# noisystreet/aither

Measured on AMD Instinct MI355X. Metric: Mcell-updates/sec per iteration (residual+LU-SGS), 256^3 block; % HBM roofline, higher is better.
Workload: dtype f64

## Files before the change

aither_amd/csrc/agx_api.hip:

```cpp
#include "agx_kernels.hpp"
#include <rccl/rccl.h>
#include <cstdarg>
#include <cstdio>
#include <cstring>
#include <cstdlib>
#include <cmath>
#include <vector>
#include <string>
#include <algorithm>

using namespace agx;

static char g_err[512] = "";
static int fail(const char* fmt, ...) {
  va_list ap;
  va_start(ap, fmt);
  vsnprintf(g_err, sizeof g_err, fmt, ap);
  va_end(ap);
  return 1;
}
#define HIPCHK(call)                                                       \
  do {                                                                     \
    hipError_t e_ = (call);                                                \
    if (e_ != hipSuccess)                                                  \
      return fail("%s failed: %s (%s:%d)", #call, hipGetErrorString(e_),   \
                  __FILE__, __LINE__);                                     \
  } while (0)
#define AGX_BY_MODE(sp, kernel, grid, block, stream, ...)                                  \
  do {                                                                                     \
    switch (agx::solver_mode_of(sp)) {                                                     \
      case 0: hipLaunchKernelGGL(kernel<0>, grid, block, 0, stream, __VA_ARGS__); break;   \
      case 1: hipLaunchKernelGGL(kernel<1>, grid, block, 0, stream, __VA_ARGS__); break;   \
      default: hipLaunchKernelGGL(kernel<2>, grid, block, 0, stream, __VA_ARGS__); break;  \
    }                                                                                      \
  } while (0)

namespace {

struct Block {
  BlockDev d;
  int global_pos = 0;
  double* slab = nullptr;
  double* d2 = nullptr;
  double* blockmat = nullptr;
  double* sweep_rec = nullptr;
  bool sweep_geo_built = false;
  bool x_planes_current = false;
  double *mg_forcing = nullptr, *mg_mres = nullptr, *mg_xsave = nullptr, *mg_nodes = nullptr;
  int* mg_tc = nullptr;
  int* mg_start = nullptr;
  double *mg_vf = nullptr, *mg_cf = nullptr;
  const void *mg_tc_key = nullptr, *mg_vf_key = nullptr, *mg_cf_key = nullptr;
  int* d2_tab = nullptr;
  std::vector<int> dstart;
  hipGraphExec_t sweep_graph[2][2][2] = {};
  int* kp_mem = nullptr;
  unsigned kp_epoch = 0;
  long d2idx(int i, int j, int k) const {
    const int ie = i + d.ng, je = j + d.ng, de = ie + je;
    return (long)(k + d.ng) * d.d2.ps + dstart[de] + je - std::max(0, de - (d.d2.Pi - 1));
  }
  bool state_is_a = true;
  agx_bc_surface* surf_dev = nullptr;
  std::vector<agx_bc_surface> surf_host;
  int* nr_off_dev = nullptr;
  double* nr_mem = nullptr;
  long nr_max = 0;
  int* wall_off_dev = nullptr;
  double* wall_mem = nullptr;
};

struct ConnSide {
  std::vector<long> h_dst, h_src;
  long n = 0;
  long* dst = nullptr;
  long* src = nullptr;
  long* dst2 = nullptr;
  long* src2 = nullptr;
};
struct Conn {
  agx_connection c;
  ConnSide side[2];
  long n_send = 0;
  long* send_src = nullptr;
  long* send_src2 = nullptr;
};

enum { G_RESID = 0, G_UPDATE = 1, G_BC = 2, G_SWEEP = 3, G_VISC = 4, G_PREPARE = 5,
       G_MRESID = 6, G_NGROUP = 7 };

// ... 26 lines not shown
  int* err_dev = nullptr;
  int* err_host = nullptr;
  double* halo_buf = nullptr;
  long halo_cap = 0;
  double* stage_buf = nullptr;
  size_t stage_cap = 0;
  double* rans_rec = nullptr;
  size_t rans_rec_cap = 0;
  bool use_gather = false;
  bool use_tile = true;
  int num_cu = 256;
  bool eager_ghosts = true;
  bool overlap = true;
  hipStream_t ov_stream = nullptr;
  hipEvent_t ov_ready = nullptr, ov_done = nullptr;
  bool visc_gather = false;
  bool visc_march = false;
  int lusgs_mode = 1;
  int spin_limit = 4000000;
  bool allow_fuse = true;
  bool fused_pending = false;
  bool use_graphs = true;
  bool sweep_records = true;
  bool sweep_three = true;
  hipStream_t cap_stream = nullptr;
  std::vector<hipStream_t> branch_streams;
  std::vector<hipEvent_t> branch_events;
  bool sweep_all_launch = true;
  BlockDev* blocks_tab = nullptr;
  BlockDev* blocks_tab_host = nullptr;
  size_t blocks_tab_n = 0;
  hipGraphExec_t sweep_graph_all[2][2][2] = {};
  bool mg_coarse = false;
  bool mres_plane_form = false;
  bool sweep_pipe = true;
  PipeJob* pipe_jobs[2] = {nullptr, nullptr};
  int* pipe_slot0 = nullptr;
  long long* pipe_progress = nullptr;
  unsigned long long* pipe_ticket = nullptr;
  size_t pipe_nblocks = 0;
  int pipe_njobs = 0, pipe_maxsteps = 0, pipe_waves = 4;
  long long pipe_launches = 0;
  bool halo_batch = true;
  bool halo_batch_required = false;
  int halo_batch_sides = 0;
  long halo_batch_nmax = 0;
  std::vector<int> halo_conn_order;
  struct HaloLevel { int first, sides; long nmax; };
  std::vector<HaloLevel> halo_levels;
  HaloSide* halo_tab_dev[5][2][2] = {};
  bool halo_tab_valid[5][2] = {};
  int halo_set[5] = {};
  HaloSide* halo_tab_host = nullptr;
  int mresid_split = 1;
  bool mresid_march = true;
  bool have_time_n = false;
  bool in_iterate = false, ghosts_prefilled = false;
  bool mres_deferred = false;
  hipEvent_t norm_event = nullptr;
  bool consn_pending = false;
  bool state_is_time_n = false;
  long fused_parts = 0;
  bool timing = false;
  std::vector<std::pair<hipEvent_t, hipEvent_t>> ev_pool;
  std::vector<std::pair<int, int>> ev_used;
  double t_ms[G_NGROUP] = {};
// ... 751 lines not shown
      }
      if (nmax > 0)
        hipLaunchKernelGGL(k_bc_faces, dim3((nmax + 255) / 256, b.nsurf), dim3(256), 0,
                           c->stream, b, c->gas, viscous, c->err_dev);
    } else {
      const long n = 4L * (b.ni + b.nj + b.nk);
      hipLaunchKernelGGL(k_bc_edges, dim3((n + 127) / 128), dim3(128), 0,
                         c->stream, b, c->gas, viscous, c->err_dev);
    }
  }
  HIPCHK(hipGetLastError());
  return 0;
}

int reduce_norms(agx_ctx* c, size_t blk_index, long nparts, NormPartial* out = nullptr) {
  if (!out) out = c->norm_out + blk_index;
  if (nparts > 4096) {
    NormPartial* tmp = c->norm_out + c->blocks.size();
    hipLaunchKernelGGL(k_norm_final, dim3(64), dim3(256), 0, c->stream, c->partials, nparts, tmp);
    hipLaunchKernelGGL(k_norm_final, dim3(1), dim3(256), 0, c->stream, tmp, 64L, out);
  } else {
    hipLaunchKernelGGL(k_norm_final, dim3(1), dim3(256), 0, c->stream,
                       c->partials, nparts, out);
  }
  HIPCHK(hipGetLastError());
  return 0;
}

int fill_ghosts(agx_ctx* c) {
  if (agx_phase_bc_faces(c)) return 1;
  if (agx_halo_exchange(c, AGX_HALO_STATE)) return 1;
  return agx_phase_bc_edges(c);
}
int update_pass(agx_ctx* c, int mode, int mm, double* l2, agx_linf* linf) {
  c->state_is_time_n = false;
  const double alpha[4] = {0.25, 1.0 / 3.0, 0.5, 1.0};
  if (mode != 2 && c->fused_pending) {
    Timer t(c, G_UPDATE);
    long off = 0;
    for (size_t n = 0; n < c->blocks.size(); ++n) {
      BlockDev& b = c->blocks[n].d;
      const MarchPlan mp = march_plan(c, b);
      hipLaunchKernelGGL(k_norm_final, dim3(1), dim3(256), 0, c->stream,
                         c->partials + off, mp.nparts, c->norm_out + n);
      off += mp.nparts;
      for (int e = 0; e < AGX_NEQ; ++e) std::swap(b.state[e], b.state2[e]);
    }
    c->halo_set[AGX_HALO_STATE] ^= 1;
    c->fused_pending = false;
    HIPCHK(hipGetLastError());
  } else {
    Timer t(c, G_UPDATE);
    for (size_t n = 0; n < c->blocks.size(); ++n) {
      const BlockDev& b = c->blocks[n].d;
      const int last = mm == c->cfg.nonlinear_iterations - 1;
#if AGX_FAST
      if (mode == 2 && b.d2.base) {
        const dim3 tg((b.ni + TT - 1) / TT, (b.nj + TT - 1) / TT, b.nk);
        hipLaunchKernelGGL(k_update_d2, tg, dim3(256), 0, c->stream, b, c->gas, c->sp, last,
                           c->partials);
        if (reduce_norms(c, n, (long)tg.x * tg.y * tg.z)) return 1;
        continue;
      }
#endif
      const dim3 grid = cell_grid(b, CELL_BLOCK);
      hipLaunchKernelGGL(k_update, grid, CELL_BLOCK, 0, c->stream, b, c->gas,
                         c->sp, mode, mode == 1 ? alpha[mm & 3] : 1.0, last,
                         c->partials);
      if (reduce_norms(c, n, (long)grid.x * grid.y * grid.z)) return 1;
    }
  }
  HIPCHK(hipMemcpyAsync(c->norm_host, c->norm_out,
                        sizeof(NormPartial) * c->blocks.size(),
                        hipMemcpyDeviceToHost, c->stream));
  if (c->mres_deferred)
    HIPCHK(hipMemcpyAsync(c->norm_host + c->blocks.size(), c->norm_out + c->blocks.size() + 64,
                          sizeof(NormPartial) * c->blocks.size(), hipMemcpyDeviceToHost,
                          c->stream));
  HIPCHK(hipMemcpyAsync(c->err_host, c->err_dev, sizeof(int),
                        hipMemcpyDeviceToHost, c->stream));
  if (c->in_iterate && c->eager_ghosts) {
    if (!c->norm_event) HIPCHK(hipEventCreateWithFlags(&c->norm_event, hipEventDisableTiming));
    HIPCHK(hipEventRecord(c->norm_event, c->stream));
    if (fill_ghosts(c)) return 1;
    c->ghosts_prefilled = true;
    HIPCHK(hipEventSynchronize(c->norm_event));
  } else {
    HIPCHK(hipStreamSynchronize(c->stream));
  }
  if (check_device_error(c)) return 1;
  for (size_t n = 0; n < c->blocks.size(); ++n) {
    const NormPartial& p = c->norm_host[n];
    const BlockDev& b = c->blocks[n].d;
// ... 24 lines not shown
  if (e != hipSuccess || ndev <= 0)
    return fail("no HIP device available (%s): the gfx950 library has no CPU "
                "path", hipGetErrorString(e));
  if (device < 0 || device >= ndev) return fail("device %d out of range", device);
  HIPCHK(hipSetDevice(device));
  agx_ctx* c = new agx_ctx();
  c->device = device;
  c->rank = rank;
  if (const char* kn = getenv("AGX_KERNEL")) {
    c->use_gather = !strcmp(kn, "gather");
    c->use_tile = !strcmp(kn, "tile");
  }
  c->allow_fuse = !(getenv("AGX_NO_FUSE") && atoi(getenv("AGX_NO_FUSE")) != 0);
  {
    int ncu = 0;
    HIPCHK(hipDeviceGetAttribute(&ncu, hipDeviceAttributeMultiprocessorCount, device));
    if (ncu > 0) c->num_cu = ncu;
    if (const char* w = getenv("AGX_WORKGROUPS")) c->num_cu = std::max(1, atoi(w));
    if (const char* w = getenv("AGX_VISC")) {
      c->visc_gather = !strcmp(w, "gather");
      c->visc_march = !strcmp(w, "march");
    }
    if (const char* w = getenv("AGX_EAGER_GHOSTS")) c->eager_ghosts = atoi(w) != 0;
    if (const char* w = getenv("AGX_OVERLAP")) c->overlap = atoi(w) != 0;
    if (const char* w = getenv("AGX_LUSGS")) c->lusgs_mode = !strcmp(w, "plane") ? 0 : 1;
    if (const char* w = getenv("AGX_SPIN_LIMIT")) c->spin_limit = std::max(1, atoi(w));
    if (const char* w = getenv("AGX_GRAPHS")) c->use_graphs = atoi(w) != 0;
    if (const char* w = getenv("AGX_SWEEP_ALL")) c->sweep_all_launch = atoi(w) != 0;
    if (const char* w = getenv("AGX_SWEEP_PIPE")) c->sweep_pipe = atoi(w) != 0;
    if (const char* w = getenv("AGX_SWEEP_THREE")) c->sweep_three = atoi(w) != 0;
    if (const char* w = getenv("AGX_SWEEP_RECORDS")) c->sweep_records = atoi(w) != 0;
    if (const char* w = getenv("AGX_MRESID_SPLIT")) c->mresid_split = std::min(64, std::max(1, atoi(w)));
    if (const char* w = getenv("AGX_MRESID")) c->mresid_march = strcmp(w, "plane") != 0;
    if (const char* w = getenv("AGX_HALO_BATCH")) {
      c->halo_batch = strcmp(w, "0") != 0;
      c->halo_batch_required = !strcmp(w, "require");
    }
  }
  HIPCHK(hipMalloc((void**)&c->err_dev, sizeof(int)));
  HIPCHK(hipMemset(c->err_dev, 0, sizeof(int)));
  HIPCHK(hipHostMalloc((void**)&c->err_host, sizeof(int)));
  *c->err_host = 0;
  *out = c;
  return 0;
}

void agx_ctx_destroy(agx_ctx* c) {
  if (!c) return;
  hipSetDevice(c->device);
  hipStreamSynchronize(c->stream);
  for (auto& b : c->blocks) {
    if (b.slab) hipFree(b.slab);
    if (b.d2) hipFree(b.d2);
    if (b.blockmat) hipFree(b.blockmat);
    if (b.sweep_rec) hipFree(b.sweep_rec);
    for (void* p : {(void*)b.mg_forcing, (void*)b.mg_mres, (void*)b.mg_xsave, (void*)b.mg_nodes,
                    (void*)b.mg_tc, (void*)b.mg_start, (void*)b.mg_vf, (void*)b.mg_cf})
      if (p) hipFree(p);
    if (b.d2_tab) hipFree(b.d2_tab);
    if (b.kp_mem) hipFree(b.kp_mem);
    for (auto& g1 : b.sweep_graph) for (auto& g2 : g1) for (auto& g3 : g2)
      if (g3) hipGraphExecDestroy(g3);
    if (b.surf_dev) hipFree(b.surf_dev);
    if (b.nr_off_dev) hipFree(b.nr_off_dev);
    if (b.nr_mem) hipFree(b.nr_mem);
    if (b.wall_off_dev) hipFree(b.wall_off_dev);
// ... 215 lines not shown
    HIPCHK(hipMemsetAsync(b.d2, 0, sizeof(double) * z.nd2 * D2_DOUBLES, c->stream));
    z.base = b.d2;
  }
  const int ci = d.ni + 2 * d.ng, cj = d.nj + 2 * d.ng, ck = d.nk + 2 * d.ng;
  if (upload_aos(c, b, g->farea_i, d.fa[0], 4, ci + 1, cj, ck, d.ng)) return 1;
  if (upload_aos(c, b, g->farea_j, d.fa[1], 4, ci, cj + 1, ck, d.ng)) return 1;
  if (upload_aos(c, b, g->farea_k, d.fa[2], 4, ci, cj, ck + 1, d.ng)) return 1;
  double* volp[1] = {d.vol};
  if (upload_aos(c, b, g->vol, volp, 1, ci, cj, ck, d.ng)) return 1;
  if (upload_aos(c, b, g->center, d.cen, 3, ci, cj, ck, d.ng)) return 1;
  const double* wsrc[3] = {g->width_i, g->width_j, g->width_k};
  for (int q = 0; q < 3; ++q) {
    double* wp[1] = {d.wid[q]};
    if (upload_aos(c, b, wsrc[q], wp, 1, ci, cj, ck, d.ng)) return 1;
  }
#if AGX_FAST
  if (d.d2.base) {
    const long n = (long)d.d2.Pi * d.d2.Pj * (d.nk + 2 * d.ng);
    hipLaunchKernelGGL(k_d2_geo, dim3((n + 255) / 256), dim3(256), 0, c->stream, d);
  }
#endif
  HIPCHK(hipGetLastError());
  if (g->wall_dist) {
    double* wp[1] = {d.wdist};
    if (upload_aos(c, b, g->wall_dist, wp, 1, ci, cj, ck, d.ng)) return 1;
  }
  *block_id = (int)c->blocks.size() - 1;
  return 0;
}

int agx_block_set_bcs(agx_ctx* c, int id, int n, const agx_bc_surface* s) {
  if (id < 0 || id >= (int)c->blocks.size()) return fail("bad block id %d", id);
  Block& b = c->blocks[id];
  for (auto& g1 : b.sweep_graph) for (auto& g2 : g1) for (auto& g3 : g2)
    if (g3) { hipGraphExecDestroy(g3); g3 = nullptr; }
  b.surf_host.assign(s, s + n);
  if (b.surf_dev) HIPCHK(hipFree(b.surf_dev));
  HIPCHK(hipMalloc((void**)&b.surf_dev, sizeof(agx_bc_surface) * (n > 0 ? n : 1)));
  HIPCHK(hipMemcpy(b.surf_dev, s, sizeof(agx_bc_surface) * n, hipMemcpyHostToDevice));
  b.d.surf = b.surf_dev;
  b.d.nsurf = n;
  b.d.nsurf_i = b.d.nsurf_j = b.d.nsurf_k = 0;
  int n_conn[6] = {0, 0, 0, 0, 0, 0}, n_other[6] = {0, 0, 0, 0, 0, 0};
  for (int q = 0; q < n; ++q) {
    const int st = surface_type(s[q]);
    if (st <= 2) b.d.nsurf_i++; else if (st <= 4) b.d.nsurf_j++; else b.d.nsurf_k++;
    const int t = s[q].bc_type;
    if (t < AGX_BC_SLIPWALL || t > AGX_BC_PERIODIC) return fail("unknown bc type %d", t);
    if (t == AGX_BC_INTERBLOCK || t == AGX_BC_PERIODIC) n_conn[st - 1]++; else n_other[st - 1]++;
    if (t == AGX_BC_VISCOUSWALL && s[q].state.is_wall_law) {
      if (AGX_NEQ == 5) return fail("wallTreatment=wallLaw needs the rans library");
    }
  }
  for (int q = 0; q < 6; ++q)
    b.d.side_conn[q] = n_conn[q] == 0 ? 0 : (n_other[q] == 0 ? 1 : 2);
  if (b.nr_off_dev) HIPCHK(hipFree(b.nr_off_dev));
  if (b.nr_mem) HIPCHK(hipFree(b.nr_mem));
  b.nr_off_dev = nullptr; b.nr_mem = nullptr; b.nr_max = 0;
  b.d.nr_off = nullptr; b.d.nr_grad = nullptr; b.d.nr_mach = nullptr;
  std::vector<int> off(n > 0 ? n : 1, -1);
  long total = 0;
  for (int q = 0; q < n; ++q) {
    const int t = s[q].bc_type;
    if (!s[q].state.is_nonreflecting || (t != AGX_BC_INLET && t != AGX_BC_PRESSURE_OUTLET)) continue;
    const int st = surface_type(s[q]);
    const int d3 = (st - 1) / 2, d1 = (d3 + 1) % 3, d2 = (d3 + 2) % 3;
// ... 131 lines not shown
      HIPCHK(hipMalloc((void**)&c->halo_tab_dev[what][set][q], sizeof(HaloSide) * sides));
  HIPCHK(hipStreamSynchronize(c->stream));
  HaloSide* g = c->halo_tab_host;
  HaloSide* p = c->halo_tab_host + sides;
  long off = 0;
  int n = 0;
  for (int cid : c->halo_conn_order) {
    auto& k = c->conns[cid];
    const agx_connection& cc = k.c;
    Block& b0 = c->blocks[cc.local_block[0]];
    Block& b1 = c->blocks[cc.local_block[1]];
    const bool z2 = halo_in_d2(b0, what);
    const long n0 = k.side[0].n, n1 = k.side[1].n;
    double* buf0 = c->halo_buf + off;
    double* buf1 = buf0 + n0 * AGX_NEQ;
    off += (n0 + n1) * AGX_NEQ;
    g[n] = HaloSide{halo_planes(b1, what), z2 ? k.side[0].src2 : k.side[0].src, n0, buf0};
    g[n + 1] = HaloSide{halo_planes(b0, what), z2 ? k.side[1].src2 : k.side[1].src, n1, buf1};
    p[n] = HaloSide{halo_planes(b0, what), z2 ? k.side[0].dst2 : k.side[0].dst, n0, buf0};
    p[n + 1] = HaloSide{halo_planes(b1, what), z2 ? k.side[1].dst2 : k.side[1].dst, n1, buf1};
    n += 2;
  }
  HIPCHK(hipMemcpyAsync(c->halo_tab_dev[what][set][0], g, sizeof(HaloSide) * sides,
                        hipMemcpyHostToDevice, c->stream));
  HIPCHK(hipMemcpyAsync(c->halo_tab_dev[what][set][1], p, sizeof(HaloSide) * sides,
                        hipMemcpyHostToDevice, c->stream));
  c->halo_tab_valid[what][set] = true;
  return 0;
}
}

int agx_setup_finalize(agx_ctx* c) {
  HIPCHK(hipSetDevice(c->device));
  const int ng = c->cfg.n_ghost;
  long max_parts = 1, max_halo = 1;
  long march_parts = 0;
  for (auto& blk : c->blocks) {
    const dim3 g = cell_grid(blk.d, CELL_BLOCK);
    max_parts = std::max(max_parts, (long)g.x * g.y * g.z);
    march_parts += march_plan(c, blk.d).nparts;
    if (blk.d.d2.base)
      max_parts = std::max(max_parts, mresid_wgs(c, blk.d));
  }
  max_parts = std::max(max_parts, march_parts);
  for (auto& k : c->conns) {
    const agx_connection& cc = k.c;
    const bool l0 = cc.rank[0] == c->rank, l1 = cc.rank[1] == c->rank;
    if (!l0 && !l1) continue;
    for (int s = 0; s < 2; ++s) {
      const bool mine = s == 0 ? l0 : l1, partner_mine = s == 0 ? l1 : l0;
      if (!mine) continue;
      const int lb = cc.local_block[s];
      if (lb < 0 || lb >= (int)c->blocks.size()) return fail("connection refers to unknown block");
      const BlockDev& br = c->blocks[lb].d;
      auto idxR = [&](int i, int j, int kk) { return br.idx(i, j, kk); };
      MapOut m;
      if (partner_mine) {
        const BlockDev& bs = c->blocks[cc.local_block[1 - s]].d;
        auto idxS = [&](int i, int j, int kk) { return bs.idx(i, j, kk); };
        build_side_map(cc, s, ng, idxR, idxS, m);
      } else {
        auto idxS = [&](int, int, int) { return 0L; };
        build_side_map(cc, s, ng, idxR, idxS, m);
        MapOut ms;
        auto idxRp = [&](int, int, int) { return 0L; };
        build_side_map(cc, 1 - s, ng, idxRp, idxR, ms);
// ... 41 lines not shown
      HIPCHK(hipHostMalloc((void**)&r.hsend, sizeof(double) * std::max<long>(r.count, 1)));
      HIPCHK(hipHostMalloc((void**)&r.hrecv, sizeof(double) * std::max<long>(r.count, 1)));
    }
    c->remote.push_back(r);
    const int s = my_side(c, c->conns[n]);
    agx_slab sl;
    sl.peer = c->conns[n].c.rank[1 - s];
    sl.tag = 0;
    bool seen = false;
    for (auto& pp : per_peer)
      if (pp.first == sl.peer) { sl.tag = pp.second++; seen = true; }
    if (!seen) per_peer.emplace_back(sl.peer, 1);
    sl.count = r.count;
    const bool hb = c->have_ex && c->ex.host_buffers;
    sl.send = hb ? r.hsend : r.send;
    sl.recv = hb ? r.hrecv : r.recv;
    c->slabs.push_back(sl);
  }
  if (c->have_ex) {
    const size_t nrec = 1 + (size_t)c->ex.nranks;
    HIPCHK(hipMalloc((void**)&c->rec_dev, sizeof(agx_ctx::NormRecord) * nrec));
    HIPCHK(hipHostMalloc((void**)&c->rec_host, sizeof(agx_ctx::NormRecord) * nrec));
  }
  c->n_partials = max_parts;
  HIPCHK(hipMalloc((void**)&c->partials, sizeof(NormPartial) * max_parts));
  const size_t nb = std::max<size_t>(c->blocks.size(), 1);
  HIPCHK(hipMalloc((void**)&c->norm_out, sizeof(NormPartial) * (2 * nb + 64)));
  HIPCHK(hipHostMalloc((void**)&c->norm_host, sizeof(NormPartial) * 2 * nb));
  c->finalized = true;
  return 0;
}

int agx_state_upload(agx_ctx* c, int id, const double* state) {
  c->ghosts_prefilled = false;
  c->state_is_time_n = false;
  if (flush_consn(c)) return 1;
  if (id < 0 || id >= (int)c->blocks.size()) return fail("bad block id %d", id);
  Block& b = c->blocks[id];
  const BlockDev& d = b.d;
  if (upload_aos(c, b, state, d.state, AGX_NEQ, d.ni + 2 * d.ng,
                 d.nj + 2 * d.ng, d.nk + 2 * d.ng, d.ng))
    return 1;
#if AGX_NEQ == 7
  hipLaunchKernelGGL(k_aux_field, dim3((d.nplane + 255) / 256), dim3(256), 0, c->stream, d,
                     c->gas, 1, d.viscp);
  HIPCHK(hipGetLastError());
#endif
  return 0;
}

static int field_info(Block& b, int field, double* const** p, int* ncomp, int* ghost) {
  BlockDev& d = b.d;
  static thread_local double* one[1];
  switch (field) {
    case AGX_FIELD_STATE: *p = d.state; *ncomp = AGX_NEQ; *ghost = 1; return 0;
    case AGX_FIELD_RESIDUAL: *p = d.resid; *ncomp = AGX_NEQ; *ghost = 0; return 0;
    case AGX_FIELD_CONS_N: *p = d.consn; *ncomp = AGX_NEQ; *ghost = 0; return 0;
    case AGX_FIELD_CONS_NM1: *p = d.consnm1; *ncomp = AGX_NEQ; *ghost = 0; return 0;
    case AGX_FIELD_UPDATE: *p = d.x; *ncomp = AGX_NEQ; *ghost = 1; return 0;
    case AGX_FIELD_DT: one[0] = d.dt; *p = one; *ncomp = 1; *ghost = 0; return 0;
    case AGX_FIELD_SPEC_RADIUS: one[0] = d.specrad; *p = one; *ncomp = 1; *ghost = 0; return 0;
    case AGX_FIELD_DIAGONAL: one[0] = d.a; *p = one; *ncomp = 1; *ghost = 0; return 0;
  }
  return 1;
}

// ... 152 lines not shown
    if (host_out[q])
      HIPCHK(hipMemcpyAsync(host_out[q], dev_out[q], sizeof(double) * count[q],
                            hipMemcpyDeviceToHost, c->stream));
  HIPCHK(hipMemcpyAsync(c->err_host, c->err_dev, sizeof(int), hipMemcpyDeviceToHost, c->stream));
  HIPCHK(hipStreamSynchronize(c->stream));
  if (*c->err_host == 4) {
    *c->err_host = 0;
    hipMemsetAsync(c->err_dev, 0, sizeof(int), c->stream);
    return fail("negative volume in PLOT3D block");
  }
  return 0;
}

int agx_nearest_wall_distance(agx_ctx* c, int64_t ncell, const double* cen, int64_t nwall,
                              const double* wall, double* dist) {
  if (ncell < 1) return 0;
  if (nwall < 1) return fail("no wall points");
  HIPCHK(hipSetDevice(c->device));
  double* buf = nullptr;
  if (stage_buffer(c, (size_t)(4 * ncell + 3 * nwall), &buf)) return 1;
  double *dc = buf, *dw = buf + 3 * ncell, *dd = dw + 3 * nwall;
  HIPCHK(hipMemcpyAsync(dc, cen, sizeof(double) * 3 * ncell, hipMemcpyHostToDevice, c->stream));
  HIPCHK(hipMemcpyAsync(dw, wall, sizeof(double) * 3 * nwall, hipMemcpyHostToDevice, c->stream));
  hipLaunchKernelGGL(k_nearest_wall, dim3((unsigned)((ncell + 255) / 256)), dim3(256), 0, c->stream,
                     (long)ncell, dc, (long)nwall, dw, dd);
  HIPCHK(hipGetLastError());
  HIPCHK(hipMemcpyAsync(dist, dd, sizeof(double) * ncell, hipMemcpyDeviceToHost, c->stream));
  HIPCHK(hipStreamSynchronize(c->stream));
  return 0;
}

int agx_field_upload(agx_ctx* c, int id, int field, const double* in) {
  x_changed(c);
  c->ghosts_prefilled = false;
  c->state_is_time_n = false;
  if (flush_consn(c)) return 1;
  if (id < 0 || id >= (int)c->blocks.size()) return fail("bad block id %d", id);
  Block& b = c->blocks[id];
  double* const* p; int nc, gh;
  if (field_info(b, field, &p, &nc, &gh)) return fail("field %d cannot be uploaded", field);
  const int g = gh ? b.d.ng : 0;
  if (upload_aos(c, b, in, p, nc, b.d.ni + 2 * g, b.d.nj + 2 * g, b.d.nk + 2 * g, g)) return 1;
  if (field == AGX_FIELD_UPDATE && b.d.d2.base) return d2_x_copy(c, b, 1);
  return 0;
}

static int implicit_begin(agx_ctx* c, int write_x);
int agx_phase_matrix_residual(agx_ctx* c, double* mr);
static int d2_x_copy(agx_ctx* c, Block& b, int to_d2);
#if AGX_FAST
static void d2_prepare(agx_ctx* c, Block& blk, int write_x, int again);
#endif
namespace {
int mg_solver_ok(agx_ctx* c) {
  if (!c->sp.implicit) return fail("multigrid: implicit time integration only");
  return 0;
}
int mg_x_to_planes(agx_ctx* c, Block& b) {
  return b.d.d2.base && !b.x_planes_current ? d2_x_copy(c, b, 0) : 0;
}
int mg_x_from_planes(agx_ctx* c, Block& b) { return b.d.d2.base ? d2_x_copy(c, b, 1) : 0; }
void mg_x_records(agx_ctx* c, Block& b) {
  if (b.d.sw_dyn)
    hipLaunchKernelGGL(k_mg_x_records, dim3((unsigned)((b.d.nplane + 255) / 256)), dim3(256), 0,
                       c->stream, b.d);
}
// ... 43 lines not shown
    b.mg_tc_key = tc;
  }
  if (vf && b.mg_vf_key != vf) {
    HIPCHK(hipStreamSynchronize(f->stream));
    if (!b.mg_vf) HIPCHK(hipMalloc((void**)&b.mg_vf, sizeof(double) * ncell));
    HIPCHK(hipMemcpy(b.mg_vf, vf, sizeof(double) * ncell, hipMemcpyHostToDevice));
    b.mg_vf_key = vf;
  }
  if (cf && b.mg_cf_key != cf) {
    HIPCHK(hipStreamSynchronize(f->stream));
    if (!b.mg_cf) HIPCHK(hipMalloc((void**)&b.mg_cf, sizeof(double) * 7 * ncell));
    HIPCHK(hipMemcpy(b.mg_cf, cf, sizeof(double) * 7 * ncell, hipMemcpyHostToDevice));
    b.mg_cf_key = cf;
  }
  if (!b.mg_tc) return fail("mg: no fine-to-coarse map for this block yet");
  m->tc = b.mg_tc;
  m->start[0] = b.mg_start;
  m->start[1] = b.mg_start + cni + 1;
  m->start[2] = m->start[1] + cnj + 1;
  m->vf = b.mg_vf;
  m->cf = b.mg_cf;
  return 0;
}
int mg_order(agx_ctx* producer, agx_ctx* consumer) {
  if (producer->stream != consumer->stream) HIPCHK(hipStreamSynchronize(producer->stream));
  return 0;
}
}

int agx_mg_restrict(agx_ctx* f, agx_ctx* cz, int blk, int what, const int32_t* tc,
                    const double* vf) {
  if (mg_check(f, cz, blk)) return 1;
  Block &bf = f->blocks[blk], &bc = cz->blocks[blk];
  if (what < AGX_MG_STATE || what > AGX_MG_FORCING) return fail("mg_restrict: bad selector %d", what);
  if (what != AGX_MG_FORCING && !vf) return fail("mg_restrict: volume weights missing");
  if (flush_consn(f) || flush_consn(cz)) return 1;
  MgMap m;
  if (mg_maps(f, bf, tc, vf, nullptr, bc.d.ni, bc.d.nj, bc.d.nk, &m)) return 1;
  if (what == AGX_MG_UPDATE && mg_x_to_planes(f, bf)) return 1;
  if (what == AGX_MG_FORCING && mg_x_to_planes(cz, bc)) return 1;
  if (mg_order(f, cz)) return 1;
  if (what == AGX_MG_STATE) {
    for (int e = 0; e < AGX_NEQ; ++e)
      HIPCHK(hipMemsetAsync(bc.d.state[e], 0, sizeof(double) * bc.d.nplane, cz->stream));
    cz->ghosts_prefilled = false;
    cz->state_is_time_n = false;
    cz->mg_coarse = true;
  } else if (what == AGX_MG_UPDATE) {
    for (int e = 0; e < AGX_NEQ; ++e)
      HIPCHK(hipMemsetAsync(bc.d.x[e], 0, sizeof(double) * bc.d.nplane, cz->stream));
  } else {
    if (!bf.d.mg_mres) return fail("mg_restrict: the fine level has no matrix residual yet");
    if (mg_planes(cz, bc, &bc.mg_forcing)) return 1;
    bc.d.mg_forcing = bc.mg_forcing;
  }
  hipLaunchKernelGGL(k_mg_restrict, cell_grid(bc.d, CELL_BLOCK), CELL_BLOCK, 0, cz->stream, bf.d,
                     bc.d, m, what);
  if (what == AGX_MG_FORCING)
    hipLaunchKernelGGL(k_mg_axmb, cell_grid(bc.d, CELL_BLOCK), CELL_BLOCK, 0, cz->stream, bc.d,
                       cz->gas, cz->sp);
  if (what == AGX_MG_UPDATE) {
    mg_x_records(cz, bc);
    if (mg_x_from_planes(cz, bc)) return 1;
  }
#if AGX_FAST
  if (what == AGX_MG_FORCING && bc.d.d2.base) d2_prepare(cz, bc, 0, 1);
#endif
  HIPCHK(hipGetLastError());
  return 0;
}

int agx_mg_matrix_residual(agx_ctx* c, double* mr) {
  if (mg_solver_ok(c)) return 1;
  for (auto& blk : c->blocks) {
    if (mg_planes(c, blk, &blk.mg_mres)) return 1;
    blk.d.mg_mres = blk.mg_mres;
    if (mg_x_to_planes(c, blk)) return 1;
  }
  c->mres_plane_form = true;
  const int rc = agx_phase_matrix_residual(c, mr);
  c->mres_plane_form = false;
  return rc;
}

int agx_mg_invert_diagonal(agx_ctx* c) { return implicit_begin(c, 0); }

int agx_mg_reset_diagonal(agx_ctx* c) {
  for (auto& blk : c->blocks) {
    HIPCHK(hipMemsetAsync(blk.d.a, 0, sizeof(double) * blk.d.nplane, c->stream));
    if (blk.d.am)
      HIPCHK(hipMemsetAsync(blk.d.am, 0, sizeof(double) * AGX_NJ * blk.d.nplane, c->stream));
    if (AGX_NEQ > 5) {
      HIPCHK(hipMemsetAsync(blk.d.a_t, 0, sizeof(double) * blk.d.nplane, c->stream));
      if (blk.d.am_t)
        HIPCHK(hipMemsetAsync(blk.d.am_t, 0, sizeof(double) * 2 * blk.d.nplane, c->stream));
    }
  }
  return 0;
}

int agx_mg_save_update(agx_ctx* c) {
  for (auto& blk : c->blocks) {
    if (mg_planes(c, blk, &blk.mg_xsave)) return 1;
    blk.d.mg_xsave = blk.mg_xsave;
    if (mg_x_to_planes(c, blk)) return 1;
    hipLaunchKernelGGL(k_mg_axpy, dim3((unsigned)((blk.d.nplane + 255) / 256)), dim3(256), 0,
                       c->stream, blk.d, 1);
  }
  HIPCHK(hipGetLastError());
  return 0;
}

int agx_mg_prolong(agx_ctx* cz, agx_ctx* f, int blk, const int32_t* tc, const double* cf) {
  if (mg_check(f, cz, blk)) return 1;
  Block &bf = f->blocks[blk], &bc = cz->blocks[blk];
  if (!bc.d.mg_xsave) return fail("mg_prolong: no saved update on the coarse level");
  if (!cf) return fail("mg_prolong: interpolation coefficients missing");
  MgMap m;
  if (mg_maps(f, bf, tc, nullptr, cf, bc.d.ni, bc.d.nj, bc.d.nk, &m)) return 1;
  const long nn = (long)(bc.d.ni + 1) * (bc.d.nj + 1) * (bc.d.nk + 1);
  if (!bc.mg_nodes) HIPCHK(hipMalloc((void**)&bc.mg_nodes, sizeof(double) * AGX_NEQ * nn));
  if (mg_x_to_planes(cz, bc) || mg_x_to_planes(f, bf)) return 1;
  hipLaunchKernelGGL(k_mg_axpy, dim3((unsigned)((bc.d.nplane + 255) / 256)), dim3(256), 0,
                     cz->stream, bc.d, 0);
  const dim3 tb = CELL_BLOCK;
  hipLaunchKernelGGL(k_mg_nodes, dim3((bc.d.ni + tb.x) / tb.x, (bc.d.nj + tb.y) / tb.y, bc.d.nk + 1),
                     tb, 0, cz->stream, bc.d, bc.mg_nodes);
  HIPCHK(hipGetLastError());
  if (mg_order(cz, f)) return 1;
  hipLaunchKernelGGL(k_mg_prolong, cell_grid(bf.d, tb), tb, 0, f->stream, bf.d, m,
                     (const double*)bc.mg_nodes, bc.d.ni, bc.d.nj, bc.d.nk);
  mg_x_records(cz, bc);
  mg_x_records(f, bf);
  if (mg_x_from_planes(cz, bc) || mg_x_from_planes(f, bf)) return 1;
  HIPCHK(hipGetLastError());
  return 0;
}

int agx_store_time_n(agx_ctx* c, int also_nm1) {
  if (flush_consn(c)) return 1;
  c->have_time_n = true;
  for (auto& blk : c->blocks)
    if (blk.nr_max > 0) c->ghosts_prefilled = false;
  static const bool lazy = !(getenv("AGX_NO_LAZY_CONSN") && atoi(getenv("AGX_NO_LAZY_CONSN")));
  c->state_is_time_n = true;
  if (lazy && !also_nm1 && !c->use_gather && all_tile_ok(c)) { c->consn_pending = true; return 0; }
  for (auto& blk : c->blocks)
    hipLaunchKernelGGL(k_store_time_n, cell_grid(blk.d, CELL_BLOCK), CELL_BLOCK,
// ... 118 lines not shown
  for (auto& blk : c->blocks)
    if (blk.nr_max > 0) {
      Timer t(c, G_BC);
      hipLaunchKernelGGL(k_nr_grads, dim3((blk.nr_max + 255) / 256, blk.d.nsurf), dim3(256), 0,
                         c->stream, blk.d, c->gas);
      HIPCHK(hipGetLastError());
    }
  return 0;
}

int agx_phase_explicit_update(agx_ctx* c, int mm, double* l2, agx_linf* linf) {
  const int mode = c->cfg.time_integration == AGX_TIME_RK4 ? 1 : 0;
  return update_pass(c, mode, mm, l2, linf);
}

static int implicit_begin(agx_ctx* c, int write_x);
#if AGX_FAST
static void d2_prepare(agx_ctx* c, Block& blk, int write_x, int again) {
  const BlockDev& b = blk.d;
  const dim3 grid((b.d2.Pi + TT - 1) / TT, (b.d2.Pj + TT - 1) / TT, b.nk + 2 * b.ng);
  hipLaunchKernelGGL(k_lusgs_prepare, grid, dim3(256), 0, c->stream, b, c->gas, c->sp,
                     write_x, write_x ? (unsigned)(++blk.kp_epoch) & 3u : 0u, again);
}
#endif
int agx_phase_implicit_begin(agx_ctx* c) { return implicit_begin(c, 1); }
static int implicit_begin(agx_ctx* c, int write_x) {
  x_changed(c);
  Timer t(c, G_PREPARE);
  c->sp.un_is_u = c->state_is_time_n ? 1 : 0;
  for (auto& blk : c->blocks) {
    const BlockDev& b = blk.d;
#if AGX_FAST
    if (b.d2.base) {
      bool conn = false;
      for (int q = 0; q < 6; ++q) conn = conn || b.side_conn[q] != 0;
      d2_prepare(c, blk, write_x && (c->sp.requires_init || conn) ? 1 : 0, 0);
      continue;
    }
#endif
    if (!c->sp.requires_init && write_x)
      hipLaunchKernelGGL(k_zero5, dim3((b.nplane + 255) / 256), dim3(256), 0,
                         c->stream, planes(b.x), b.nplane);
    hipLaunchKernelGGL(k_implicit_begin, cell_grid(b, CELL_BLOCK), CELL_BLOCK, 0,
                       c->stream, b, c->gas, c->sp, c->err_dev, write_x);
    if (b.sw_geo) {
      hipLaunchKernelGGL(k_sweep_records, dim3((unsigned)((b.nplane + 255) / 256)), dim3(256), 0,
                         c->stream, b, c->sp, blk.sweep_geo_built ? 0 : 1);
      blk.sweep_geo_built = true;
    }
  }
  HIPCHK(hipGetLastError());
  return 0;
}

int agx_phase_relax_forward(agx_ctx* c, int sweep) {
  x_changed(c);
  Timer t(c, G_SWEEP);
  const int full = sweep > 0 || c->sp.requires_init;
  bool swept = false;
  if (is_lusgs_solver(c) && pipe_sweep_applicable(c)) return lusgs_sweep_pipe(c, true, full);
  if (is_lusgs_solver(c) && plane_sweep_all_applicable(c)) return lusgs_sweep_all(c, true, full);
  for (auto& blk : c->blocks) {
    BlockDev& b = blk.d;
    if (is_lusgs_solver(c)) {
      if (lusgs_sweep(c, blk, true, full)) return 1;
      swept = true;
    } else {
      for (int e = 0; e < AGX_NEQ; ++e) std::swap(b.x[e], b.xold[e]);
      AGX_BY_MODE(c->sp, k_dplur, cell_grid(b, CELL_BLOCK), CELL_BLOCK, c->stream, b, c->gas,
// ... 437 lines not shown
```

aither_amd/csrc/agx_lusgs_kernels.hpp:

```cpp
#pragma once

namespace agx {

constexpr int TT = 32;
constexpr int TRS = TT + 2;
__device__ __forceinline__ int tile_diag_index(int li, int lj) {
  const int dd = li + lj;
  if (dd < TT) return dd * (dd + 1) / 2 + lj;
  const int r = 2 * TT - 2 - dd;
  return TT * TT - (r + 1) * (r + 2) / 2 + (lj - (dd - (TT - 1)));
}
__device__ __forceinline__ void tile_table(unsigned short* s_tab) {
  const int tid = threadIdx.x;
#pragma unroll
  for (int m = 0; m < 4; ++m) {
    const int li = tid & (TT - 1), lj = (tid >> 5) + 8 * m;
    s_tab[tile_diag_index(li, lj)] = (unsigned short)(li | (lj << 8));
  }
}

__device__ __forceinline__ double kp_tagged(double v, unsigned tag) {
  const unsigned long long u = (unsigned long long)__double_as_longlong(v);
  return __longlong_as_double((long long)((u & ~3ull) | tag));
}
// ... 16 lines not shown
#pragma unroll
  for (int d = 0; d < 3; ++d) {
    double a[4];
#pragma unroll
    for (int c = 0; c < 4; ++c) a[c] = b.fa[d][c][q];
    double ad = 0.0;
    if (e3[d] > 0) {
      const long ql = q - b.stride(d);
      const double v[3] = {b.cen[0][q] - b.cen[0][ql], b.cen[1][q] - b.cen[1][ql],
                           b.cen[2][q] - b.cen[2][ql]};
      const double dist = dot3(v, a);
      ad = dist != 0.0 ? a[3] / dist : 0.0;
    }
    z.pa(PA_F + 2 * d + 0)[p] = make_double2(a[0], a[1]);
    z.pa(PA_F + 2 * d + 1)[p] = make_double2(a[2], a[3]);
    z.ad(d)[p] = ad;
  }
}
__global__ void __launch_bounds__(256) k_d2_x_copy(BlockDev b, int to_d2, unsigned tag) {
  const D2Dev& z = b.d2;
  const long t = (long)blockIdx.x * blockDim.x + threadIdx.x;
  const long n = (long)z.Pi * z.Pj * (b.nk + 2 * b.ng);
  if (t >= n) return;
  const int ie = (int)(t % z.Pi), je = (int)((t / z.Pi) % z.Pj),
            ke = (int)(t / ((long)z.Pi * z.Pj));
  const long q = b.idx(ie - b.ng, je - b.ng, ke - b.ng);
  const long p = (long)ke * z.ps + z.pos2(ie, je);
#pragma unroll
  for (int e = 0; e < AGX_NEQ; ++e) {
    double* xp = reinterpret_cast<double*>(z.pa(PA_X + (e >> 1))) + 2 * p + (e & 1);
    if (to_d2) *xp = kp_tagged(b.x[e][q], tag);
    else b.x[e][q] = *xp;
  }
}

__global__ void __launch_bounds__(256)
k_lusgs_prepare(BlockDev b, GasDev g, SolverDev sp, int write_x, unsigned tag, int again) {
  __shared__ double sv[6][TT][TRS];
  __shared__ unsigned short s_tab[TT * TT];
  const D2Dev& z = b.d2;
  const int tid = threadIdx.x;
  tile_table(s_tab);
  const int i0 = blockIdx.x * TT, j0 = blockIdx.y * TT, ke = blockIdx.z;
  const int k = ke - b.ng;
  const int li = tid & (TT - 1);
  double bb[4][AGX_NEQ], x0[4][AGX_NEQ], ainv[4], vf[4];
#pragma unroll
  for (int m = 0; m < 4; ++m) {
    const int lj = (tid >> 5) + 8 * m;
    const int ie = i0 + li, je = j0 + lj;
    const int i = ie - b.ng, j = je - b.ng;
#pragma unroll
    for (int e = 0; e < AGX_NEQ; ++e) { bb[m][e] = 0.0; x0[m][e] = 0.0; }
    ainv[m] = 1.0;
    vf[m] = 0.0;
    double cs = 0.0;
    if (ie < z.Pi && je < z.Pj) {
      const long q = b.idx(i, j, k);
      double s[AGX_NEQ];
#pragma unroll
      for (int e = 0; e < AGX_NEQ; ++e) { s[e] = b.state[e][q]; sv[e][lj][li] = s[e]; }
      if (s[0] > 0.0) cs = sound_speed(g, s);
      if (sp.viscous) vf[m] = cell_visc_factor(g, s);
      const bool phys = i >= 0 && i < b.ni && j >= 0 && j < b.nj && k >= 0 && k < b.nk;
      if (phys) {
        double dvt = (b.vol[q] * (1.0 + sp.zeta)) / (b.dt[q] * sp.theta);
        if (sp.dual_time_cfl > 0.0) dvt += fmax(b.specrad[q], 0.0) / sp.dual_time_cfl;
        const double a = again ? b.ainv[q] : b.a[q] * sp.relax + dvt;
        b.ainv[q] = a;
        if (sp.diag_add) b.a[q] = a;
        ainv[m] = 1.0 / a;
        rhs_bf(b, g, sp, q, bb[m]);
        if (sp.requires_init) {
#pragma unroll
          for (int e = 0; e < AGX_NEQ; ++e) x0[m][e] = bb[m][e] * ainv[m];
        }
      }
    }
    sv[5][lj][li] = cs;
  }
  __syncthreads();
  long pos[4];
  int tli[4], tlj[4];
#pragma unroll
  for (int m = 0; m < 4; ++m) {
    const unsigned tl = s_tab[tid + 256 * m];
    tli[m] = tl & 0xff; tlj[m] = tl >> 8;
    const int ie = i0 + tli[m], je = j0 + tlj[m];
    pos[m] = -1;
    if (ie < z.Pi && je < z.Pj) {
      pos[m] = (long)ke * z.ps + z.pos2(ie, je);
#pragma unroll
      for (int h = 0; h < 3; ++h)
        z.pa(PA_S + h)[pos[m]] = make_double2(sv[2 * h][tlj[m]][tli[m]], sv[2 * h + 1][tlj[m]][tli[m]]);
    }
  }
  __syncthreads();
#pragma unroll
  for (int m = 0; m < 4; ++m) {
    const int lj = (tid >> 5) + 8 * m;
#pragma unroll
    for (int e = 0; e < AGX_NEQ; ++e) sv[e][lj][li] = bb[m][e];
    sv[5][lj][li] = ainv[m];
  }
  __syncthreads();
  double ai2[4];
#pragma unroll
  for (int m = 0; m < 4; ++m) {
    ai2[m] = sv[5][tlj[m]][tli[m]];
    if (pos[m] >= 0) {
#pragma unroll
      for (int h = 0; h < 3; ++h)
        z.pa(PA_B + h)[pos[m]] = make_double2(sv[2 * h][tlj[m]][tli[m]], sv[2 * h + 1][tlj[m]][tli[m]]);
    }
  }
  __syncthreads();
#pragma unroll
  for (int m = 0; m < 4; ++m) {
    const int lj = (tid >> 5) + 8 * m;
#pragma unroll
    for (int e = 0; e < AGX_NEQ; ++e) sv[e][lj][li] = x0[m][e];
    sv[5][lj][li] = vf[m];
  }
  __syncthreads();
#pragma unroll
  for (int m = 0; m < 4; ++m) {
    if (pos[m] >= 0) {
      if (write_x) {
        z.pa(PA_X + 0)[pos[m]] = make_double2(kp_tagged(sv[0][tlj[m]][tli[m]], tag),
                                              kp_tagged(sv[1][tlj[m]][tli[m]], tag));
        z.pa(PA_X + 1)[pos[m]] = make_double2(kp_tagged(sv[2][tlj[m]][tli[m]], tag),
                                              kp_tagged(sv[3][tlj[m]][tli[m]], tag));
        z.pa(PA_X + 2)[pos[m]] = make_double2(kp_tagged(sv[4][tlj[m]][tli[m]], tag), ai2[m]);
      }
      if (sp.viscous) z.vf()[pos[m]] = sv[5][tlj[m]][tli[m]];
    }
  }
}

struct KpRec {
  double dx[AGX_NEQ];
  double r1, v1[3], p1, h1;
  double r0, v0[3], p0, h0;
  double cs, vf;
};
constexpr int KP_NV = 19;
template <class G>
__device__ __forceinline__ void kp_build_rec(const G& g, const double* s, double cs,
                                             double vf, const double* dx, KpRec& r) {
  const double ke = g.hf + 0.5 * dot3(s + 1, s + 1);
  const double e0 = s[0] * ke + g.n * s[4];
  r.r0 = s[0]; r.p0 = s[4]; r.h0 = e0 + s[4]; r.cs = cs; r.vf = vf;
  const double r1 = s[0] + dx[0];
  const double ir = fast_rcp(r1);
  double v2 = 0.0;
#pragma unroll
  for (int q = 0; q < 3; ++q) {
    r.v0[q] = s[1 + q];
    r.v1[q] = fma(s[0], s[1 + q], dx[1 + q]) * ir;
    v2 = fma(r.v1[q], r.v1[q], v2);
  }
  const double e1 = e0 + dx[4];
  r.r1 = r1;
  r.p1 = (e1 - r1 * (g.hf + 0.5 * v2)) * g.inv_n;
  r.h1 = e1 + r.p1;
#pragma unroll
  for (int e = 0; e < AGX_NEQ; ++e) r.dx[e] = dx[e];
}
// ... 432 lines not shown
      KpFace ff;
      if (i > 0 || bc_is_connection(b, i, j, k, 1)) {
        kp_load_face(z, 0, own, visc, ff);
        kp_term_mem(z, g, visc, kbase + qlo, ff, true, acc);
      }
      if (j > 0 || bc_is_connection(b, i, j, k, 3)) {
        kp_load_face(z, 1, own, visc, ff);
        kp_term_mem(z, g, visc, kbase + qlo - 1, ff, true, acc);
      }
      if (k > 0 || bc_is_connection(b, i, j, k, 5)) col_term(cm, fk0, true, acc);
      if (i < b.ni - 1 || bc_is_connection(b, i + 1, j, k, 2)) {
        kp_load_face(z, 0, kbase + qup, visc, ff);
        kp_term_mem(z, g, visc, kbase + qup, ff, false, acc);
      }
      if (j < b.nj - 1 || bc_is_connection(b, i, j + 1, k, 4)) {
        kp_load_face(z, 1, kbase + qup + 1, visc, ff);
        kp_term_mem(z, g, visc, kbase + qup + 1, ff, false, acc);
      }
      if (k < b.nk - 1 || bc_is_connection(b, i, j, k + 1, 6)) col_term(cp, fk1, false, acc);
      const double a = 1.0 / b2.y;
      const double bv[AGX_NEQ] = {b0.x, b0.y, b1.x, b1.y, b2.x};
#pragma unroll
      for (int e = 0; e < AGX_NEQ; ++e) {
        const double r = -(c0.x[e] * a - acc[e] - bv[e]);
        l2[e] += r * r;
      }
      cm = c0; c0 = cp; fk0 = fk1;
    }
  }
  norm_block_fold(l2, -1.0e300, 0x7fffffffffffffffLL, partials + blockIdx.x);
}

__global__ void __launch_bounds__(256)
k_update_d2(BlockDev b, GasDev g, SolverDev sp, int last_mm, NormPartial* partials) {
  __shared__ double sv[AGX_NEQ][TT][TRS];
  __shared__ unsigned short s_tab[TT * TT];
  const D2Dev& z = b.d2;
  const int tid = threadIdx.x;
  tile_table(s_tab);
  __syncthreads();
  const int i0 = blockIdx.x * TT, j0 = blockIdx.y * TT, k = blockIdx.z;
#pragma unroll
  for (int m = 0; m < 4; ++m) {
    const unsigned tl = s_tab[tid + 256 * m];
    const int tli = tl & 0xff, tlj = tl >> 8;
    const int i = i0 + tli, j = j0 + tlj;
    if (i < b.ni && j < b.nj) {
      const long p = (long)(k + b.ng) * z.ps + z.pos2(i + b.ng, j + b.ng);
      const double2 x0 = z.pa(PA_X)[p], x1 = z.pa(PA_X + 1)[p], x2 = z.pa(PA_X + 2)[p];
      sv[0][tlj][tli] = x0.x; sv[1][tlj][tli] = x0.y; sv[2][tlj][tli] = x1.x;
      sv[3][tlj][tli] = x1.y; sv[4][tlj][tli] = x2.x;
    }
  }
  __syncthreads();
  const int li = tid & (TT - 1);
  double l2[AGX_NEQ] = {0, 0, 0, 0, 0};
  double vmax = -1.0e300;
  long long vlin = 0x7fffffffffffffffLL;
#pragma unroll
  for (int m = 0; m < 4; ++m) {
    const int lj = (tid >> 5) + 8 * m;
    const int i = i0 + li, j = j0 + lj;
    if (i < b.ni && j < b.nj) {
      const long q = b.idx(i, j, k);
      double r[AGX_NEQ], s[AGX_NEQ], du[AGX_NEQ], ns[AGX_NEQ];
      load5(b.resid, q, r);
      load5(b.state, q, s);
#pragma unroll
      for (int e = 0; e < AGX_NEQ; ++e) du[e] = sv[e][lj][li];
      update_prim_with_cons(g, s, du, ns);
      store5(b.state, q, ns);
      if (sp.bdf2 && last_mm) {
        double u[AGX_NEQ];
        load5(b.consn, q, u);
        store5(b.consnm1, q, u);
      }
      const long lin0 = (((long)k * b.nj + j) * b.ni + i) * AGX_NEQ;
#pragma unroll
      for (int e = 0; e < AGX_NEQ; ++e) {
        l2[e] += r[e] * r[e];
        if (r[e] > vmax || (r[e] == vmax && lin0 + e < vlin)) { vmax = r[e]; vlin = lin0 + e; }
      }
    }
  }
  const long bid = ((long)blockIdx.z * gridDim.y + blockIdx.y) * gridDim.x + blockIdx.x;
  norm_block_fold(l2, vmax, vlin, partials + bid);
}

}
```

Measured before the change: 1458.

## Fuse diagonal-plane state write into update and add lean LU-SGS prepare

The update kernel now also writes the new primitive state, sound speed and viscous factor into the diagonal-plane (d2) layout when the block qualifies. This lets the following LU-SGS prepare step run a lean kernel that only computes the RHS and inverse diagonal instead of re-gathering the state. The aim is to avoid a separate full prepare pass that rereads state from memory. Validity flags track when the d2 state is fresh, and the inverse diagonal is recomputed lazily on multigrid paths. The cost is more bookkeeping and a risk of using stale d2 data if a flag is not reset on some path that changes the state.

```diff
diff --git a/aither_amd/csrc/agx_api.hip b/aither_amd/csrc/agx_api.hip
--- a/aither_amd/csrc/agx_api.hip
+++ b/aither_amd/csrc/agx_api.hip
@@ -56,6 +56,8 @@
   hipGraphExec_t sweep_graph[2][2][2] = {};
   int* kp_mem = nullptr;
   unsigned kp_epoch = 0;
+  bool d2_state_ok = false;
+  bool ainv_stale = false;
   long d2idx(int i, int j, int k) const {
     const int ie = i + d.ng, je = j + d.ng, de = ie + je;
     return (long)(k + d.ng) * d.d2.ps + dstart[de] + je - std::max(0, de - (d.d2.Pi - 1));
@@ -148,6 +150,8 @@
   size_t blocks_tab_n = 0;
   hipGraphExec_t sweep_graph_all[2][2][2] = {};
   bool mg_coarse = false;
+  bool prepare_full = false;
+  bool mg_level = false;
   bool mres_plane_form = false;
   bool sweep_pipe = true;
   PipeJob* pipe_jobs[2] = {nullptr, nullptr};
@@ -965,8 +969,20 @@
   if (agx_halo_exchange(c, AGX_HALO_STATE)) return 1;
   return agx_phase_bc_edges(c);
 }
+void d2_state_stale(agx_ctx* c) {
+  for (auto& blk : c->blocks) blk.d2_state_ok = false;
+}
+bool lean_prepare_ok(const agx_ctx* c, const Block& blk) {
+  const BlockDev& b = blk.d;
+  if (!b.d2.base || c->prepare_full || c->mg_coarse || c->mg_level || c->sp.requires_init)
+    return false;
+  for (int q = 0; q < 6; ++q)
+    if (b.side_conn[q] != 0) return false;
+  return true;
+}
 int update_pass(agx_ctx* c, int mode, int mm, double* l2, agx_linf* linf) {
   c->state_is_time_n = false;
+  if (mode != 2) d2_state_stale(c);
   const double alpha[4] = {0.25, 1.0 / 3.0, 0.5, 1.0};
   if (mode != 2 && c->fused_pending) {
     Timer t(c, G_UPDATE);
@@ -987,11 +1003,14 @@
     for (size_t n = 0; n < c->blocks.size(); ++n) {
       const BlockDev& b = c->blocks[n].d;
       const int last = mm == c->cfg.nonlinear_iterations - 1;
+      c->blocks[n].d2_state_ok = false;
 #if AGX_FAST
       if (mode == 2 && b.d2.base) {
         const dim3 tg((b.ni + TT - 1) / TT, (b.nj + TT - 1) / TT, b.nk);
+        const int wd2 = lean_prepare_ok(c, c->blocks[n]) ? 1 : 0;
         hipLaunchKernelGGL(k_update_d2, tg, dim3(256), 0, c->stream, b, c->gas, c->sp, last,
-                           c->partials);
+                           wd2, c->partials);
+        c->blocks[n].d2_state_ok = wd2 != 0;
         if (reduce_norms(c, n, (long)tg.x * tg.y * tg.z)) return 1;
         continue;
       }
@@ -1082,6 +1101,7 @@
     if (const char* w = getenv("AGX_SWEEP_RECORDS")) c->sweep_records = atoi(w) != 0;
     if (const char* w = getenv("AGX_MRESID_SPLIT")) c->mresid_split = std::min(64, std::max(1, atoi(w)));
     if (const char* w = getenv("AGX_MRESID")) c->mresid_march = strcmp(w, "plane") != 0;
+    if (const char* w = getenv("AGX_PREPARE")) c->prepare_full = !strcmp(w, "full");
     if (const char* w = getenv("AGX_HALO_BATCH")) {
       c->halo_batch = strcmp(w, "0") != 0;
       c->halo_batch_required = !strcmp(w, "require");
@@ -1363,6 +1383,7 @@
 int agx_block_set_bcs(agx_ctx* c, int id, int n, const agx_bc_surface* s) {
   if (id < 0 || id >= (int)c->blocks.size()) return fail("bad block id %d", id);
   Block& b = c->blocks[id];
+  b.d2_state_ok = false;
   for (auto& g1 : b.sweep_graph) for (auto& g2 : g1) for (auto& g3 : g2)
     if (g3) { hipGraphExecDestroy(g3); g3 = nullptr; }
   b.surf_host.assign(s, s + n);
@@ -1560,6 +1581,7 @@
 
 int agx_setup_finalize(agx_ctx* c) {
   HIPCHK(hipSetDevice(c->device));
+  d2_state_stale(c);
   const int ng = c->cfg.n_ghost;
   long max_parts = 1, max_halo = 1;
   long march_parts = 0;
@@ -1667,6 +1689,7 @@
 }
 
 int agx_state_upload(agx_ctx* c, int id, const double* state) {
+  d2_state_stale(c);
   c->ghosts_prefilled = false;
   c->state_is_time_n = false;
   if (flush_consn(c)) return 1;
@@ -1885,6 +1908,7 @@
 
 int agx_field_upload(agx_ctx* c, int id, int field, const double* in) {
   x_changed(c);
+  d2_state_stale(c);
   c->ghosts_prefilled = false;
   c->state_is_time_n = false;
   if (flush_consn(c)) return 1;
@@ -1994,6 +2018,7 @@
                     const double* vf) {
   if (mg_check(f, cz, blk)) return 1;
   Block &bf = f->blocks[blk], &bc = cz->blocks[blk];
+  d2_state_stale(cz);
   if (what < AGX_MG_STATE || what > AGX_MG_FORCING) return fail("mg_restrict: bad selector %d", what);
   if (what != AGX_MG_FORCING && !vf) return fail("mg_restrict: volume weights missing");
   if (flush_consn(f) || flush_consn(cz)) return 1;
@@ -2034,10 +2059,17 @@
 
 int agx_mg_matrix_residual(agx_ctx* c, double* mr) {
   if (mg_solver_ok(c)) return 1;
+  c->mg_level = true;
   for (auto& blk : c->blocks) {
     if (mg_planes(c, blk, &blk.mg_mres)) return 1;
     blk.d.mg_mres = blk.mg_mres;
     if (mg_x_to_planes(c, blk)) return 1;
+#if AGX_FAST
+    if (blk.ainv_stale) {
+      d2_prepare(c, blk, 0, 0);
+      blk.ainv_stale = false;
+    }
+#endif
   }
   c->mres_plane_form = true;
   const int rc = agx_phase_matrix_residual(c, mr);
@@ -2076,6 +2108,8 @@
 int agx_mg_prolong(agx_ctx* cz, agx_ctx* f, int blk, const int32_t* tc, const double* cf) {
   if (mg_check(f, cz, blk)) return 1;
   Block &bf = f->blocks[blk], &bc = cz->blocks[blk];
+  d2_state_stale(f);
+  d2_state_stale(cz);
   if (!bc.d.mg_xsave) return fail("mg_prolong: no saved update on the coarse level");
   if (!cf) return fail("mg_prolong: interpolation coefficients missing");
   MgMap m;
@@ -2260,9 +2294,17 @@
     const BlockDev& b = blk.d;
 #if AGX_FAST
     if (b.d2.base) {
+      if (write_x && blk.d2_state_ok && lean_prepare_ok(c, blk)) {
+        const dim3 tg((b.ni + TT - 1) / TT, (b.nj + TT - 1) / TT, b.nk);
+        hipLaunchKernelGGL(k_lusgs_prepare_lean, tg, dim3(256), 0, c->stream, b, c->gas, c->sp,
+                           0);
+        blk.ainv_stale = true;
+        continue;
+      }
       bool conn = false;
       for (int q = 0; q < 6; ++q) conn = conn || b.side_conn[q] != 0;
       d2_prepare(c, blk, write_x && (c->sp.requires_init || conn) ? 1 : 0, 0);
+      blk.ainv_stale = false;
       continue;
     }
 #endif
diff --git a/aither_amd/csrc/agx_lusgs_kernels.hpp b/aither_amd/csrc/agx_lusgs_kernels.hpp
--- a/aither_amd/csrc/agx_lusgs_kernels.hpp
+++ b/aither_amd/csrc/agx_lusgs_kernels.hpp
@@ -72,6 +72,18 @@
     if (to_d2) *xp = kp_tagged(b.x[e][q], tag);
     else b.x[e][q] = *xp;
   }
+}
+
+__device__ __forceinline__ void prepare_cell(const BlockDev& b, const GasDev& g,
+                                             const SolverDev& sp, long q, int again,
+                                             bool store_ainv, double* bb, double& ainv) {
+  double dvt = (b.vol[q] * (1.0 + sp.zeta)) / (b.dt[q] * sp.theta);
+  if (sp.dual_time_cfl > 0.0) dvt += fmax(b.specrad[q], 0.0) / sp.dual_time_cfl;
+  const double a = again ? b.ainv[q] : b.a[q] * sp.relax + dvt;
+  if (store_ainv) b.ainv[q] = a;
+  if (sp.diag_add) b.a[q] = a;
+  ainv = 1.0 / a;
+  rhs_bf(b, g, sp, q, bb);
 }
 
 __global__ void __launch_bounds__(256)
@@ -104,13 +116,7 @@
       if (sp.viscous) vf[m] = cell_visc_factor(g, s);
       const bool phys = i >= 0 && i < b.ni && j >= 0 && j < b.nj && k >= 0 && k < b.nk;
       if (phys) {
-        double dvt = (b.vol[q] * (1.0 + sp.zeta)) / (b.dt[q] * sp.theta);
-        if (sp.dual_time_cfl > 0.0) dvt += fmax(b.specrad[q], 0.0) / sp.dual_time_cfl;
-        const double a = again ? b.ainv[q] : b.a[q] * sp.relax + dvt;
-        b.ainv[q] = a;
-        if (sp.diag_add) b.a[q] = a;
-        ainv[m] = 1.0 / a;
-        rhs_bf(b, g, sp, q, bb[m]);
+        prepare_cell(b, g, sp, q, again, true, bb[m], ainv[m]);
         if (sp.requires_init) {
 #pragma unroll
           for (int e = 0; e < AGX_NEQ; ++e) x0[m][e] = bb[m][e] * ainv[m];
@@ -174,6 +180,42 @@
         z.pa(PA_X + 2)[pos[m]] = make_double2(kp_tagged(sv[4][tlj[m]][tli[m]], tag), ai2[m]);
       }
       if (sp.viscous) z.vf()[pos[m]] = sv[5][tlj[m]][tli[m]];
+    }
+  }
+}
+
+__global__ void __launch_bounds__(256)
+k_lusgs_prepare_lean(BlockDev b, GasDev g, SolverDev sp, int store_ainv) {
+  __shared__ double sv[6][TT][TRS];
+  __shared__ unsigned short s_tab[TT * TT];
+  const D2Dev& z = b.d2;
+  const int tid = threadIdx.x;
+  tile_table(s_tab);
+  const int i0 = blockIdx.x * TT, j0 = blockIdx.y * TT, k = blockIdx.z;
+  const int li = tid & (TT - 1);
+#pragma unroll
+  for (int m = 0; m < 4; ++m) {
+    const int lj = (tid >> 5) + 8 * m;
+    const int i = i0 + li, j = j0 + lj;
+    if (i < b.ni && j < b.nj) {
+      double bb[AGX_NEQ], ainv;
+      prepare_cell(b, g, sp, b.idx(i, j, k), 0, store_ainv != 0, bb, ainv);
+#pragma unroll
+      for (int e = 0; e < AGX_NEQ; ++e) sv[e][lj][li] = bb[e];
+      sv[5][lj][li] = ainv;
+    }
+  }
+  __syncthreads();
+#pragma unroll
+  for (int m = 0; m < 4; ++m) {
+    const unsigned tl = s_tab[tid + 256 * m];
+    const int tli = tl & 0xff, tlj = tl >> 8;
+    const int i = i0 + tli, j = j0 + tlj;
+    if (i < b.ni && j < b.nj) {
+      const long p = (long)(k + b.ng) * z.ps + z.pos2(i + b.ng, j + b.ng);
+#pragma unroll
+      for (int h = 0; h < 3; ++h)
+        z.pa(PA_B + h)[p] = make_double2(sv[2 * h][tlj][tli], sv[2 * h + 1][tlj][tli]);
     }
   }
 }
@@ -672,7 +714,8 @@
 }
 
 __global__ void __launch_bounds__(256)
-k_update_d2(BlockDev b, GasDev g, SolverDev sp, int last_mm, NormPartial* partials) {
+k_update_d2(BlockDev b, GasDev g, SolverDev sp, int last_mm, int write_d2,
+            NormPartial* partials) {
   __shared__ double sv[AGX_NEQ][TT][TRS];
   __shared__ unsigned short s_tab[TT * TT];
   const D2Dev& z = b.d2;
@@ -710,6 +753,8 @@
       for (int e = 0; e < AGX_NEQ; ++e) du[e] = sv[e][lj][li];
       update_prim_with_cons(g, s, du, ns);
       store5(b.state, q, ns);
+#pragma unroll
+      for (int e = 0; e < AGX_NEQ; ++e) sv[e][lj][li] = ns[e];
       if (sp.bdf2 && last_mm) {
         double u[AGX_NEQ];
         load5(b.consn, q, u);
@@ -723,6 +768,27 @@
       }
     }
   }
+  if (write_d2) {
+    __syncthreads();
+#pragma unroll
+    for (int m = 0; m < 4; ++m) {
+      const unsigned tl = s_tab[tid + 256 * m];
+      const int tli = tl & 0xff, tlj = tl >> 8;
+      const int i = i0 + tli, j = j0 + tlj;
+      if (i < b.ni && j < b.nj) {
+        const long p = (long)(k + b.ng) * z.ps + z.pos2(i + b.ng, j + b.ng);
+        double s[AGX_NEQ];
+#pragma unroll
+        for (int e = 0; e < AGX_NEQ; ++e) s[e] = sv[e][tlj][tli];
+        double cs = 0.0;
+        if (s[0] > 0.0) cs = sound_speed(g, s);
+        z.pa(PA_S + 0)[p] = make_double2(s[0], s[1]);
+        z.pa(PA_S + 1)[p] = make_double2(s[2], s[3]);
+        z.pa(PA_S + 2)[p] = make_double2(s[4], cs);
+        if (sp.viscous) z.vf()[p] = cell_visc_factor(g, s);
+      }
+    }
+  }
   const long bid = ((long)blockIdx.z * gridDim.y + blockIdx.y) * gridDim.x + blockIdx.x;
   norm_block_fold(l2, vmax, vlin, partials + bid);
 }
```

Result: faster. 1475, median of 6 (+1.2%).
